# federicobetti99/Conjugate-Gradient

Hardware: AMD Instinct MI355X
Metric: cg_iterations_per_sec (higher is better)
Workload: dtype f64

## Files before the change

conjugate-gradient_amd/cgx.py:

```python
import ctypes as C
import os
import subprocess
import sys

import numpy as np

_PKG = os.path.dirname(os.path.abspath(__file__))
LIB_PATH = os.path.join(_PKG, "libcgx.so")
UNIQUE_ID_BYTES = 128

IPC_HANDLE_BYTES = 64
COMM_SELF, COMM_LOOPBACK, COMM_RCCL, COMM_P2P = 0, 1, 2, 3
MATRIX_DENSE, MATRIX_BANDED = 0, 1
MATRIX_CSR = 2
MAX_DIAGONALS = 64

EXPORTS = [
    "cgx_config_init", "cgx_comm_unique_id", "cgx_create", "cgx_destroy", "cgx_last_error", "cgx_status_string",
    "cgx_get_comm_info", "cgx_get_gemv_plan", "cgx_get_resident_record", "cgx_p2p_export", "cgx_p2p_import", "cgx_p2p_selftest",
    "cgx_partition", "cgx_generate_lap2d_matrix", "cgx_set_matrix_dense", "cgx_read_matrix",
    "cgx_init_source_term", "cgx_set_source_term", "cgx_set_max_iter", "cgx_set_tolerance", "cgx_get_size",
    "cgx_get_matrix_format",
    "cgx_solve", "cgx_solve_begin", "cgx_solve_steps", "cgx_solve_end", "cgx_get_gemv_samples",
    "cgx_get_update_samples",
    "cgx_probe_gemv", "cgx_probe_time_gemv", "cgx_probe_vector_ops", "cgx_probe_get_matrix_rows",
    "cgx_probe_get_source_term", "cgx_probe_set_fault_after", "cgx_probe_set_resident_limit", "cgx_probe_persistent_plan",
    "cgx_probe_parse_matrix_market", "cgx_probe_p2p_mailbox_to_host", "cgx_probe_fill_matrix_hash",
    "cgx_probe_set_p2p_epoch", "cgx_probe_get_p2p_epoch", "cgx_probe_p2p_host_mailboxes", "cgx_probe_resident_test",
    "cgx_solve_multi", "cgx_probe_gemv_multi",
    "cgx_set_preconditioner", "cgx_get_preconditioner",
    "cgx_set_matrix_csr", "cgx_get_matrix_nnz",
]
MAX_RHS = 16
PRECOND_NONE, PRECOND_JACOBI = 0, 1
_PRECOND_NAMES = {None: PRECOND_NONE, "jacobi": PRECOND_JACOBI}


class Config(C.Structure):
    _fields_ = [
        ("struct_version", C.c_int), ("comm_mode", C.c_int), ("device", C.c_int), ("rank", C.c_int),
        ("nranks", C.c_int), ("unique_id", C.c_ubyte * UNIQUE_ID_BYTES), ("gemv_variant", C.c_int),
        ("lda_pad", C.c_int), ("check_every", C.c_int), ("profile_gemv", C.c_int), ("profile_update", C.c_int),
        ("p2p_mailbox_kib", C.c_int), ("p2p_timeout_ms", C.c_int), ("p2p_separate_exchange", C.c_int),
        ("matrix_format", C.c_int), ("profile_first", C.c_int), ("profile_markers", C.c_int),
        ("p2p_no_acquire_fence", C.c_int), ("p2p_tagged", C.c_int),
    ]
# ... 72 lines not shown
        L.cgx_get_matrix_nnz.argtypes = [vp, C.c_int, C.POINTER(C.c_longlong)]
        L.cgx_solve.argtypes = [vp, dp, C.POINTER(Result)]
        L.cgx_solve_begin.argtypes = [vp, dp]
        L.cgx_solve_steps.argtypes = [vp, C.c_int, ip]
        L.cgx_solve_end.argtypes = [vp, dp, C.POINTER(Result)]
        L.cgx_get_gemv_samples.argtypes = [vp, dp, C.c_int, ip]
        L.cgx_get_update_samples.argtypes = [vp, dp, C.c_int, ip]
        L.cgx_probe_gemv.argtypes = [vp, dp, dp, dp]
        L.cgx_probe_time_gemv.argtypes = [vp, C.c_int, dp]
        L.cgx_probe_vector_ops.argtypes = [vp, C.c_int, C.c_double, C.c_double, dp, dp, dp, dp, dp]
        L.cgx_probe_get_matrix_rows.argtypes = [vp, C.c_int, dp, ip, ip]
        L.cgx_probe_get_source_term.argtypes = [vp, C.c_int, dp]
        L.cgx_probe_set_fault_after.argtypes = [vp, C.c_int]
        L.cgx_probe_set_resident_limit.argtypes = [vp, C.c_int]
        L.cgx_probe_persistent_plan.argtypes = [C.c_int, C.c_int, C.c_long, C.c_int, C.POINTER(C.c_long)]
        L.cgx_probe_p2p_mailbox_to_host.argtypes = [vp]
        L.cgx_probe_fill_matrix_hash.argtypes = [vp, C.c_ulonglong, C.c_int, C.c_double]
        L.cgx_probe_p2p_host_mailboxes.argtypes = [vp, C.c_char_p, C.c_int]
        L.cgx_probe_set_p2p_epoch.argtypes = [vp, C.c_int, C.c_ulonglong]
        L.cgx_probe_resident_test.argtypes = [vp, C.c_ulonglong, C.c_int]
        L.cgx_probe_get_p2p_epoch.argtypes = [vp, C.c_int, C.POINTER(C.c_ulonglong)]
        L.cgx_solve_multi.argtypes = [vp, C.c_int, dp, C.c_long, dp, C.c_long, C.POINTER(Result)]
        L.cgx_set_preconditioner.argtypes = [vp, C.c_int]
        L.cgx_get_preconditioner.argtypes = [vp, ip]
        L.cgx_probe_gemv_multi.argtypes = [vp, C.c_int, dp, C.c_long, dp, C.c_long, dp]
        L.cgx_probe_parse_matrix_market.argtypes = [C.c_char_p, C.c_int, ip, ip, ip, ip, ip, ip, dp, C.c_long, C.c_char_p, C.c_int]
        for name in EXPORTS:
            fn = getattr(L, name)
            if fn.restype is C.c_int and name not in ("cgx_config_init",):
                fn.restype = C.c_int
# ... 322 lines not shown
```

conjugate-gradient_amd/csrc/cgx_context.cpp:

```cpp
#include "cgx_internal.h"

#include <sys/mman.h>
#include <sys/stat.h>
#include <fcntl.h>
#include <unistd.h>

#include <algorithm>
#include <cctype>
#include <chrono>
#include <cmath>
#include <cstdio>
#include <cstdlib>
#include <cstring>
#include <string>
#include <vector>

using namespace cgxi;

namespace cgxi {

constexpr int kStreamDefaultMax = 10000;

thread_local std::string g_create_error;

// ... 43 lines not shown
    (void)hipFree(s.A);
    (void)hipFree(s.dia_vals);
    (void)hipFree(s.csr_rp);
    (void)hipFree(s.csr_col);
    (void)hipFree(s.csr_vals);
    (void)hipFree(s.b_full);
    (void)hipFree(s.x);
    (void)hipFree(s.p[0]);
    (void)hipFree(s.p[1]);
    (void)hipFree(s.apg);
    (void)hipFree(s.rbuf);
    (void)hipFree(s.partials);
    (void)hipFree(s.ap_parts);
    (void)hipFree(s.k1_scratch);
    (void)hipFree(s.sym_parts);
    (void)hipFree(s.dinv);
    (void)hipFree(s.zbuf);
    (void)hipFree(s.sc);
    (void)hipFree(s.gathered);
    s = Shard{};
}

void free_problem(cgx_ctx *ctx)
{
    for (auto &s : ctx->shards) free_shard(s);
    ctx->shards.clear();
    (void)hipFree(ctx->d_gathered_ptrs);
    (void)hipFree(ctx->d_scalar_ptrs);
    (void)hipFree(ctx->multi);
    ctx->multi = nullptr;
// ... 129 lines not shown
        ctx->max_iter = n;
        ctx->have_matrix = ctx->have_b = false;
        ctx->in_solve = false;
        for (auto &s : ctx->shards) {
            HIP_TRY(ctx, hipMemsetAsync(s.p[0], 0, (size_t)ctx->lda * sizeof(double), ctx->stream));
            HIP_TRY(ctx, hipMemsetAsync(s.p[1], 0, (size_t)ctx->lda * sizeof(double), ctx->stream));
            HIP_TRY(ctx, hipMemsetAsync(s.sc, 0, sizeof(Scalars), ctx->stream));
            HIP_TRY(ctx, hipMemsetAsync(s.apg, 0, (size_t)ctx->nranks * ctx->seg_S * sizeof(double), ctx->stream));
        }
        {
            int variant = ctx->cfg.gemv_variant;
            if (variant <= 0) {
                const char *e = getenv("CGX_GEMV_VARIANT");
                if (e) variant = atoi(e);
            }
            CGX_TRY(setup_resident(ctx, variant));
        }
        HIP_TRY(ctx, hipStreamSynchronize(ctx->stream));
        return CGX_OK;
    }
    free_problem(ctx);
    ctx->m = ctx->n = n;
    if (n <= (8 << 20) &&
        hipHostMalloc(reinterpret_cast<void **>(&ctx->h_stage), (size_t)(n + 16) * sizeof(double), hipHostMallocDefault) != hipSuccess)
        ctx->h_stage = nullptr;
    ctx->max_iter = n;
    ctx->lda = default_lda(ctx, n);
    ctx->start_rows.assign(ctx->nranks, 0);
    ctx->num_rows.assign(ctx->nranks, 0);
    partition_rows(n, ctx->nranks, ctx->start_rows.data(), ctx->num_rows.data());
    int max_rows = 0;
    for (int q = 0; q < ctx->nranks; ++q) max_rows = std::max(max_rows, ctx->num_rows[q]);
    ctx->seg_Sr = std::max((max_rows + 1) / 2 * 2, 2);

    int variant = ctx->cfg.gemv_variant;
    if (variant <= 0) {
        const char *e = getenv("CGX_GEMV_VARIANT");
        if (e) variant = atoi(e);
    }
    const bool fused_p2p = ctx->cfg.comm_mode == CGX_COMM_P2P && !ctx->cfg.p2p_separate_exchange;
    ctx->chunked = (ctx->nranks > 1 && !ctx->sparse()) || fused_p2p;
    const bool allow_split = ctx->chunked && !ctx->sparse() && ctx->nranks > 1;
    const int k1_variant = (variant == 40000 || variant == 50000) ? 0 : variant;
    auto plan_for = [&](int rows) {
        if (ctx->csr) return cgx::plan_csr(rows, 0, k1_variant);
        return ctx->banded ? cgx::plan_dia(rows, k1_variant) : cgx::plan_gemv(k1_variant, rows, ctx->n, ctx->lda, allow_split);
    };
    int grid_max = 1;
    for (int q = 0; q < ctx->nranks; ++q) {
        const cgx::GemvPlan pl = plan_for(ctx->num_rows[q]);
        grid_max = std::max(grid_max, pl.grid);
        if (pl.split > 1) ctx->chunked = true;
    }
    const int cpr = cgx::chunks_per_rank(ctx->seg_Sr);
// ... 38 lines not shown
    const int seg_tail = (ctx->npart + 1 + 1) / 2 * 2;
    ctx->seg_S = ctx->seg_Sr + seg_tail;
    const int nlocal = (ctx->cfg.comm_mode == CGX_COMM_LOOPBACK) ? ctx->nranks : 1;
    ctx->shards.resize(nlocal);
    for (int i = 0; i < nlocal; ++i) {
        Shard &s = ctx->shards[i];
        s.rank = (ctx->cfg.comm_mode == CGX_COMM_RCCL || ctx->cfg.comm_mode == CGX_COMM_P2P) ? ctx->cfg.rank : i;
        s.row0 = ctx->start_rows[s.rank];
        s.rows = ctx->num_rows[s.rank];
        s.plan = plan_for(s.rows);
        const size_t rows_alloc = (size_t)std::max(s.rows, 1);
        s.npartials = 3 * cgx::update_xr_grid(n) + 8;
        if (!ctx->sparse()) HIP_TRY(ctx, hipMalloc(&s.A, rows_alloc * (size_t)ctx->lda * sizeof(double)));
        HIP_TRY(ctx, hipMalloc(&s.b_full, (size_t)n * sizeof(double)));
        const size_t apg_bytes = (size_t)ctx->nranks * ctx->seg_S * sizeof(double);
        const int rr_parts = cgx::update_xr_grid(n);
        const size_t rbuf_bytes = (size_t)(ctx->lda + rr_parts) * sizeof(double);
        const bool blocks = ctx->cfg.comm_mode == CGX_COMM_SELF && !ctx->sparse();
        HIP_TRY(ctx, hipMalloc(&s.p[0], (size_t)ctx->lda * sizeof(double)));
        if (blocks) {
            static_assert(sizeof(Scalars) <= 16 * sizeof(double), "Scalars must fit the tail of a state block");
            const size_t bytes = (size_t)cgx::state_doubles(ctx->lda) * sizeof(double);
            for (int q = 0; q < 2; ++q) {
                HIP_TRY(ctx, hipMalloc(&s.state[q], bytes));
                HIP_TRY(ctx, hipMemsetAsync(s.state[q], 0, bytes, ctx->stream));
            }
            s.cur = 0;
            bind_state(s, ctx->lda);
        } else {
            HIP_TRY(ctx, hipMalloc(&s.x, rows_alloc * sizeof(double)));
            HIP_TRY(ctx, hipMalloc(&s.p[1], (size_t)ctx->lda * sizeof(double)));
// ... 39 lines not shown
    }
    HIP_TRY(ctx, hipStreamSynchronize(ctx->stream));
    return CGX_OK;
}

cgx_status plan_symmetric(cgx_ctx *ctx)
{
    ctx->dinv_valid = false;
    if (ctx->shards.size() != 1 || ctx->nranks != 1 || ctx->sparse() || ctx->chunked) return CGX_OK;
    Shard &s = ctx->shards[0];
    int variant = ctx->cfg.gemv_variant;
    if (variant <= 0) {
        const char *e = getenv("CGX_GEMV_VARIANT");
        if (e) variant = atoi(e);
    }
    const int k1_variant = (variant == 40000 || variant == 50000) ? 0 : variant;
    const cgx::GemvPlan general = cgx::plan_gemv(k1_variant, s.rows, ctx->n, ctx->lda, false);
    const cgx::GemvPlan sym = cgx::plan_symv(ctx->n, ctx->lda, ctx->cus);
    const bool eligible = variant <= 0 && ctx->n > cgx::kSymvMinN && s.rows == ctx->n && s.A && sym.light <= ctx->npart;
    if (!eligible) {
        s.plan = general;
        return CGX_OK;
    }
    DeviceScratch scratch;
    int *dflag = nullptr;
    HIP_TRY(ctx, scratch.alloc(&dflag, sizeof(int)));
    HIP_TRY(ctx, hipMemsetAsync(dflag, 0, sizeof(int), ctx->stream));
    HIP_TRY(ctx, cgx::launch_symmetric_check(s.A, ctx->lda, ctx->n, dflag, ctx->stream));
    int mismatch = 1;
    HIP_TRY(ctx, hipMemcpyAsync(&mismatch, dflag, sizeof(int), hipMemcpyDeviceToHost, ctx->stream));
    HIP_TRY(ctx, hipStreamSynchronize(ctx->stream));
    if (mismatch) {
        s.plan = general;
        return CGX_OK;
    }
    const size_t bytes = (size_t)sym.split * (size_t)ctx->lda * sizeof(double);
    if (s.sym_parts && s.sym_parts_bytes != bytes) {
        (void)hipFree(s.sym_parts);
        s.sym_parts = nullptr;
        s.sym_parts_bytes = 0;
    }
    if (!s.sym_parts) {
        HIP_TRY(ctx, hipMalloc(&s.sym_parts, bytes));
        s.sym_parts_bytes = bytes;
        HIP_TRY(ctx, hipMemsetAsync(s.sym_parts, 0, bytes, ctx->stream));
        HIP_TRY(ctx, hipStreamSynchronize(ctx->stream));
    }
    s.plan = sym;
    return CGX_OK;
}

}

extern "C" {

void cgx_config_init(cgx_config *cfg)
{
    if (!cfg) return;
    memset(cfg, 0, sizeof *cfg);
    cfg->struct_version = CGX_VERSION;
    cfg->comm_mode = CGX_COMM_SELF;
// ... 433 lines not shown
```

conjugate-gradient_amd/csrc/cgx_internal.h:

```cpp
#pragma once

#include "../../include/cgx.h"

#include <hip/hip_runtime.h>

#include <string>
#include <vector>

#include "cgx_kernels.h"
#include "cgx_rccl.h"

namespace cgxi {

using cgx::Scalars;

struct Shard {
    int rank = 0;
    int row0 = 0;
    int rows = 0;
    double *A = nullptr;
    double *dia_vals = nullptr;
    cgx::DiaView dia{};
    long long *csr_rp = nullptr;
    int *csr_col = nullptr;
    double *csr_vals = nullptr;
    cgx::CsrView csr{};
    double *b_full = nullptr;
    double *state[2] = {nullptr, nullptr};
    int cur = 0;
    double *x = nullptr;
    double *p[2] = {nullptr, nullptr};
    double *apg = nullptr;
    double *rbuf = nullptr;
    double *ap_parts = nullptr;
    double *k1_scratch = nullptr;
    double *partials = nullptr;
    double *sym_parts = nullptr;
    size_t sym_parts_bytes = 0;
    Scalars *sc = nullptr;
    double *gathered = nullptr;
    cgx::GemvPlan plan{};
    cgx::SegView apv{}, rv{};
    double *dinv = nullptr;
    double *zbuf = nullptr;
    cgx::SegView zv{};
    int npartials = 0;
    double *Ap() const { return apg + (size_t)rank * apv.S; }
    double *tail() const { return Ap() + apv.Sr; }
    double *k1_part() const { return k1_scratch ? k1_scratch : tail(); }
};


}
// ... 207 lines not shown
```

conjugate-gradient_amd/csrc/cgx_kernels.h:

```cpp
#pragma once

#include <hip/hip_runtime.h>

namespace cgx {

constexpr int kSlots = 4;
constexpr int kSlotConj = 0;
constexpr int kSlotRr = 1;
constexpr int kSlotX = 2;
constexpr int kMaxRanks = 64;

struct Scalars {
    double rs[2];
    double rr[2];
    double local[kSlots];
    double dbg[4];
    int    done;
    int    k_final;
    unsigned pad[2];
};

struct SegView {
    double *base;
    int S, Sr;
// ... 6 lines not shown
};

void seg_finalize(SegView *sv);

struct GemvPlan {
    int variant;
    int R;
    int U;
    int waves;
    int nt;
    int grid;
    int rows_per_wg;
    int ncols;
    int split;
    int light;
};

GemvPlan plan_gemv(int variant, int rows, int n, long lda, bool allow_split = false);

hipError_t launch_gemv_plain(const GemvPlan &plan, const double *A, long lda, int rows, const double *v_full,
                             const double *v_local, double *Ap, double *partials, Scalars *sc, hipStream_t s);

hipError_t launch_gemv_fused(const GemvPlan &plan, const double *A, long lda, int rows, int row0,
                             const double *p_old, double *p_new, SegView seg, double *Ap, double *partials,
                             Scalars *sc, int k, double tol, hipStream_t s, hipEvent_t e_start = nullptr,
                             hipEvent_t e_stop = nullptr, long ap_stride = 0, bool jacobi = false);
constexpr int kSymvTile = 256;
constexpr int kSymvMinN = 16384;
GemvPlan plan_symv(int n, long lda, int cus);
inline int plan_partials(const GemvPlan &pl) { return pl.variant == 6 ? pl.light : pl.grid / (pl.split > 1 ? pl.split : 1); }
hipError_t launch_symv_plain(const GemvPlan &pl, const double *A, long lda, int n, const double *v, double *parts, double *Ap,
                             double *partials, hipStream_t s);
hipError_t launch_symv_fused(const GemvPlan &pl, const double *A, long lda, int n, const double *p_old, double *p_new, SegView seg,
                             double *parts, double *Ap, double *partials, Scalars *sc, int k, double tol, hipStream_t s,
                             hipEvent_t e_start = nullptr, hipEvent_t e_stop = nullptr, bool jacobi = false);
hipError_t launch_symmetric_check(const double *A, long lda, int n, int *mismatch, hipStream_t s);

constexpr int kChunkRows = 512;
inline int chunks_per_rank(int Sr) { return (Sr + kChunkRows - 1) / kChunkRows; }
hipError_t launch_prefold_ap(const double *parts, int split, long stride, int rows, int Sr, const double *p_loc, double *dst,
                             double *tail, const Scalars *sc, hipStream_t s);

hipError_t launch_update_xr(int n, int rows, int row0, const double *p_new, SegView apv, int tail_off, int tail_count,
                            double *x, SegView rv, Scalars *sc, int parity, double *partials, hipStream_t s,
                            hipEvent_t e_start = nullptr, hipEvent_t e_stop = nullptr,
                            const double *dinv = nullptr, SegView zv = SegView{});
int update_xr_grid(int count);
constexpr int kMaxVectorGrid = 1024;

hipError_t launch_close_iteration(Scalars *sc, SegView seg, int k, double tol, hipStream_t s, bool jacobi = false);
// ... 203 lines not shown
```

conjugate-gradient_amd/csrc/cgx_probe.cpp:

```cpp
#include "cgx_internal.h"

#include <fcntl.h>
#include <sys/mman.h>
#include <sys/stat.h>
#include <unistd.h>

#include <algorithm>
#include <cctype>
#include <chrono>
#include <cmath>
#include <cstdio>
#include <cstdlib>
#include <cstring>
#include <string>
#include <vector>

using namespace cgxi;

extern "C" {

cgx_status cgx_probe_gemv(cgx_ctx *ctx, const double *p, double *y, double *pAp)
{
    if (!ctx || !p || !y) return fail(ctx, CGX_ERR_BAD_ARG, "cgx_probe_gemv: bad argument");
    if (!ctx->have_matrix) return fail(ctx, CGX_ERR_BAD_ARG, "no matrix");
// ... 238 lines not shown
    ctx->p2p_ready = true;
    return CGX_OK;
}

cgx_status cgx_probe_persistent_plan(int n, int cus, long lds_per_cu, int streaming, long out[CGX_PERSISTENT_PLAN_INTS])
{
    if (!out || n < 1 || cus < 1 || lds_per_cu < 0) return CGX_ERR_BAD_ARG;
    cgx::ResidentPlan pl{};
    const bool fits = streaming ? cgx::plan_stream(n, cus, (size_t)lds_per_cu, &pl) : cgx::plan_resident(n, cus, (size_t)lds_per_cu, &pl);
    const long r[CGX_PERSISTENT_PLAN_INTS] = {fits ? 1 : 0, pl.R, pl.S, pl.grid, pl.xslots, (long)pl.lds_bytes, pl.RL, pl.RG, pl.RB, pl.l2_rows,
                                              pl.hybrid, pl.stream ? 512 : 256};
    for (int i = 0; i < CGX_PERSISTENT_PLAN_INTS; ++i) out[i] = fits || i == 0 ? r[i] : 0;
    return CGX_OK;
}

cgx_status cgx_probe_set_resident_limit(cgx_ctx *ctx, int workgroups)
{
    if (!ctx) return CGX_ERR_BAD_ARG;
    ctx->resident_limit = workgroups;
    return CGX_OK;
}

cgx_status cgx_probe_get_source_term(cgx_ctx *ctx, int local_shard, double *b_out)
{
    if (!ctx || !b_out || local_shard < 0 || local_shard >= (int)ctx->shards.size())
        return fail(ctx, CGX_ERR_BAD_ARG, "cgx_probe_get_source_term: bad argument");
    if (!ctx->have_b) return fail(ctx, CGX_ERR_BAD_ARG, "no source term");
    HIP_TRY(ctx, hipSetDevice(ctx->device));
    HIP_TRY(ctx, hipMemcpy(b_out, ctx->shards[local_shard].b_full, (size_t)ctx->n * sizeof(double), hipMemcpyDeviceToHost));
    return CGX_OK;
// ... 55 lines not shown
```

conjugate-gradient_amd/csrc/cgx_solve.cpp:

```cpp
#include "cgx_internal.h"

#include <sys/file.h>

#include <cerrno>
#include <climits>
#include <thread>

#include <algorithm>
#include <cctype>
#include <chrono>
#include <cmath>
#include <cstdio>
#include <cstdlib>
#include <cstring>
#include <string>
#include <vector>

using namespace cgxi;

namespace cgxi {


cgx_status p2p_allgather(cgx_ctx *ctx, int chan, const double *src, int count, double *dst, long dst_stride,
                         int copy_self, int tail_off, int tail_n, int sum_off)
// ... 60 lines not shown
cgx_status prepare_jacobi(cgx_ctx *ctx)
{
    if (ctx->banded) return fail(ctx, CGX_ERR_UNSUPPORTED, "Jacobi preconditioner: banded storage is not supported");
    if (ctx->res_forced)
        return fail(ctx, CGX_ERR_UNSUPPORTED, "Jacobi preconditioner: the persistent kernels (gemv_variant 40000 / 50000) have no Jacobi form");
    hipStream_t st = ctx->stream;
    for (auto &s : ctx->shards) {
        if (!s.dinv) {
            const size_t zbytes = (size_t)(s.rv.S + (s.rv.S - s.rv.Sr)) * sizeof(double);
            HIP_TRY(ctx, hipMalloc(&s.dinv, (size_t)ctx->lda * sizeof(double)));
            HIP_TRY(ctx, hipMalloc(&s.zbuf, zbytes));
            HIP_TRY(ctx, hipMemsetAsync(s.zbuf, 0, zbytes, st));
        }
        s.zv = s.rv;
        s.zv.base = s.zbuf;
    }
    if (ctx->dinv_valid) return CGX_OK;
    for (auto &s : ctx->shards) {
        if (ctx->csr)
            HIP_TRY(ctx, cgx::launch_csr_diag_slice(s.csr, s.rows, s.row0, s.Ap(), st));
        else
            HIP_TRY(ctx, cgx::launch_diag_slice(s.A, ctx->lda, s.rows, s.row0, s.Ap(), st));
    }
    CGX_TRY(gather_segments(ctx, false));
    if (!ctx->d_jbad) HIP_TRY(ctx, hipMalloc(reinterpret_cast<void **>(&ctx->d_jbad), sizeof(int)));
    HIP_TRY(ctx, hipMemsetAsync(ctx->d_jbad, 0x7f, sizeof(int), st));
    for (auto &s : ctx->shards) HIP_TRY(ctx, cgx::launch_jacobi_dinv(s.apv, ctx->n, ctx->lda, s.dinv, ctx->d_jbad, st));
    int bad = INT_MAX;
    HIP_TRY(ctx, hipMemcpyAsync(&bad, ctx->d_jbad, sizeof(int), hipMemcpyDeviceToHost, st));
    HIP_TRY(ctx, hipStreamSynchronize(st));
// ... 39 lines not shown
    *e1 = ctx->upd_pool[ctx->upd_used++];
    return CGX_OK;
}

}

namespace cgxi {

cgx_status run_gemv_plain(cgx_ctx *ctx, Shard &s, const double *v_full)
{
    if (ctx->csr)
        HIP_TRY(ctx, cgx::launch_spmv_csr_plain(s.plan, s.csr, s.rows, s.row0, ctx->lda, v_full, s.Ap(), s.k1_part(), ctx->stream));
    else if (ctx->banded)
        HIP_TRY(ctx, cgx::launch_spmv_dia_plain(s.plan, s.dia, s.rows, s.row0, ctx->n, ctx->lda, v_full, s.Ap(), s.k1_part(), s.sc,
                                                ctx->stream));
    else if (s.plan.variant == 6)
        HIP_TRY(ctx, cgx::launch_symv_plain(s.plan, s.A, ctx->lda, ctx->n, v_full, s.sym_parts, s.Ap(), s.k1_part(), ctx->stream));
    else
        HIP_TRY(ctx, cgx::launch_gemv_plain(s.plan, s.A, ctx->lda, s.rows, v_full, v_full + s.row0, s.Ap(), s.k1_part(),
                                            s.sc, ctx->stream));
    return CGX_OK;
}

cgx_status run_gemv_fused(cgx_ctx *ctx, Shard &s, int k)
{
    const int every = ctx->cfg.profile_gemv;
    const long long seq = ctx->gemv_seq++;
    bool timed = false;
    if (every > 0 && ctx->ev_used + 2 <= 4096) {
        if (seq == 0) {
// ... 9 lines not shown
        CGX_TRY(take_event(ctx, &e0));
        CGX_TRY(take_event(ctx, &e1));
        if (ctx->cfg.profile_markers) {
            HIP_TRY(ctx, hipEventRecord(e0, ctx->stream));
            e0 = e1 = nullptr;
        }
    }
    hipEvent_t m1 = (timed && ctx->cfg.profile_markers) ? ctx->ev_pool[ctx->ev_used - 1] : nullptr;
    const bool pc = ctx->precond == CGX_PRECOND_JACOBI;
    if (ctx->csr)
        HIP_TRY(ctx, cgx::launch_spmv_csr_fused(s.plan, s.csr, s.rows, s.row0, ctx->lda, s.p[k & 1], s.p[(k + 1) & 1], pc ? s.zv : s.rv,
                                                s.Ap(), s.k1_part(), s.sc, k, ctx->tol, ctx->stream, e0, e1, pc));
    else if (ctx->banded)
        HIP_TRY(ctx, cgx::launch_spmv_dia_fused(s.plan, s.dia, s.rows, s.row0, ctx->n, ctx->lda, s.p[k & 1], s.p[(k + 1) & 1],
                                                s.rv, s.Ap(), s.k1_part(), s.sc, k, ctx->tol, ctx->stream, e0, e1));
    else if (s.plan.variant == 6)
        HIP_TRY(ctx, cgx::launch_symv_fused(s.plan, s.A, ctx->lda, ctx->n, s.p[k & 1], s.p[(k + 1) & 1], pc ? s.zv : s.rv, s.sym_parts,
                                            s.Ap(), s.k1_part(), s.sc, k, ctx->tol, ctx->stream, e0, e1, pc));
    else
        HIP_TRY(ctx, cgx::launch_gemv_fused(s.plan, s.A, ctx->lda, s.rows, s.row0, s.p[k & 1], s.p[(k + 1) & 1], pc ? s.zv : s.rv,
                                            s.plan.split > 1 ? s.ap_parts : s.Ap(),
                                            (ctx->chunked && s.plan.light) ? nullptr : s.k1_part(),
                                            s.sc, k, ctx->tol, ctx->stream, e0, e1, ctx->seg_Sr, pc));
    if (m1) HIP_TRY(ctx, hipEventRecord(m1, ctx->stream));
    return CGX_OK;
}

void reset_gemv_stats(cgx_ctx *ctx)
{
    ctx->ev_used = 0;
// ... 49 lines not shown
        HIP_TRY(ctx, cgx::launch_update_xr_p2p(ctx->n, s.rows, s.row0, s.p[(k + 1) & 1], s.apv, ctx->npart, ctx->mv, 1, epoch,
                                               s.x, s.rv, s.sc, k & 1, ctx->p2p_timeout_ticks, ctx->d_p2p_err, st,
                                               s.plan.split > 1 ? s.ap_parts : s.Ap(), s.plan.split, ctx->seg_Sr, u0, u1,
                                               pc ? s.dinv : nullptr, s.zv));
        return CGX_OK;
    }
    if (ctx->chunked)
        for (auto &s : ctx->shards)
            HIP_TRY(ctx, cgx::launch_prefold_ap(s.plan.split > 1 ? s.ap_parts : s.Ap(), s.plan.split, ctx->seg_Sr, s.rows, ctx->seg_Sr,
                                                s.p[(k + 1) & 1] + s.row0, s.Ap(), s.tail(), s.sc, st));
    CGX_TRY(gather_segments(ctx, true));
    const bool folded = ctx->cfg.comm_mode == CGX_COMM_P2P;
    for (auto &s : ctx->shards) {
        hipEvent_t u0 = nullptr, u1 = nullptr;
        if (&s == &ctx->shards[0]) CGX_TRY(take_update_events(ctx, &u0, &u1));
        const int count = folded ? 1 : (s.plan.variant == 6 ? cgx::plan_partials(s.plan) : ctx->npart);
        HIP_TRY(ctx, cgx::launch_update_xr(ctx->n, s.rows, s.row0, s.p[(k + 1) & 1], s.apv, folded ? ctx->npart : 0,
                                           count, s.x, s.rv, s.sc, k & 1, s.partials, st, u0, u1,
                                           pc ? s.dinv : nullptr, s.zv));
    }
    return CGX_OK;
}

cgx_status check_p2p_error(cgx_ctx *ctx)
{
    if (ctx->cfg.comm_mode != CGX_COMM_P2P || !ctx->d_p2p_err) return CGX_OK;
    int e = 0;
    HIP_TRY(ctx, hipMemcpy(&e, ctx->d_p2p_err, sizeof(int), hipMemcpyDeviceToHost));
    if (e) return fail(ctx, CGX_ERR_P2P, "direct peer exchange: a wait for a peer's flag expired (peer dead or IPC not coherent)");
    return CGX_OK;
// ... 443 lines not shown
```

include/cgx.h:

```cpp
#ifndef CGX_H
#define CGX_H

#ifdef __cplusplus
extern "C" {
#endif

#define CGX_VERSION 1
#define CGX_UNIQUE_ID_BYTES 128
#define CGX_IPC_HANDLE_BYTES 64

typedef enum cgx_status {
    CGX_OK = 0,
    CGX_ERR_BAD_ARG = 1,
    CGX_ERR_IO = 2,
    CGX_ERR_HIP = 3,
    CGX_ERR_RCCL = 4,
    CGX_ERR_OOM = 5,
    CGX_ERR_NO_DEVICE = 6,
    CGX_ERR_UNSUPPORTED = 7,
    CGX_ERR_P2P = 8
} cgx_status;

typedef enum cgx_comm_mode {
    CGX_COMM_SELF = 0,
// ... 103 lines not shown
cgx_status  cgx_solve_multi(cgx_ctx *ctx, int nrhs, const double *B, long ldb, double *X, long ldx, cgx_result *res);
cgx_status  cgx_probe_gemv_multi(cgx_ctx *ctx, int nrhs, const double *P, long ldp, double *Y, long ldy, double *pAp);

cgx_status  cgx_probe_gemv(cgx_ctx *ctx, const double *p, double *y, double *pAp);
cgx_status  cgx_probe_time_gemv(cgx_ctx *ctx, int reps, double *ms_per_launch);
cgx_status  cgx_probe_vector_ops(cgx_ctx *ctx, int n, double alpha, double beta, double *x, double *r,
                                 double *p, const double *Ap, double *rr);
cgx_status  cgx_probe_set_fault_after(cgx_ctx *ctx, int calls);
cgx_status  cgx_probe_parse_matrix_market(const char *path, int threads, int *m, int *n, int *nz, int *symmetric, int *I, int *J,
                                          double *a, long cap, char *err, int err_cap);
cgx_status  cgx_probe_p2p_mailbox_to_host(cgx_ctx *ctx);
cgx_status  cgx_probe_p2p_host_mailboxes(cgx_ctx *ctx, const char *prefix, int stage);
cgx_status  cgx_probe_set_resident_limit(cgx_ctx *ctx, int workgroups);
#define CGX_PERSISTENT_PLAN_INTS 12
cgx_status  cgx_probe_persistent_plan(int n, int cus, long lds_per_cu, int streaming, long out[CGX_PERSISTENT_PLAN_INTS]);
cgx_status  cgx_probe_set_p2p_epoch(cgx_ctx *ctx, int chan, unsigned long long value);
cgx_status  cgx_probe_get_p2p_epoch(cgx_ctx *ctx, int chan, unsigned long long *value);
cgx_status  cgx_probe_resident_test(cgx_ctx *ctx, unsigned long long epoch, int mute_workgroup);
cgx_status  cgx_probe_get_source_term(cgx_ctx *ctx, int local_shard, double *b_out);
cgx_status  cgx_probe_fill_matrix_hash(cgx_ctx *ctx, unsigned long long seed, int symmetric, double diag);
cgx_status  cgx_probe_get_matrix_rows(cgx_ctx *ctx, int local_shard, double *A_out, int *row0, int *rows);

#ifdef __cplusplus
}
#endif
#endif
```

Before: 1369.

## Add evenly balanced symmetric SYMV tile schedule with fold-into-update kernel

Adds a new symmetric matrix-vector path that splits the upper-triangle tile work into equal-length step runs across a fixed grid of four workgroups per CU, so no workgroup gets a heavier share. Tiles that are cut between workgroups write their column sums to an extras buffer, looked up through a host-built table. The x/r update kernel then folds the per-strip partial results directly, removing a separate reduction pass. This is the default for single-rank dense problems above the size threshold, with variant 60000 keeping the old chain path. The price is extra buffers and more complex indexing, plus correctness risk around tiles that are split between workgroups.

After: 1369. About the same (-0.0%).

```diff
diff --git a/conjugate-gradient_amd/cgx.py b/conjugate-gradient_amd/cgx.py
--- a/conjugate-gradient_amd/cgx.py
+++ b/conjugate-gradient_amd/cgx.py
@@ -30,6 +30,7 @@
     "cgx_solve_multi", "cgx_probe_gemv_multi",
     "cgx_set_preconditioner", "cgx_get_preconditioner",
     "cgx_set_matrix_csr", "cgx_get_matrix_nnz",
+    "cgx_probe_symv_even_plan",
 ]
 MAX_RHS = 16
 PRECOND_NONE, PRECOND_JACOBI = 0, 1
@@ -132,6 +133,7 @@
         L.cgx_probe_set_fault_after.argtypes = [vp, C.c_int]
         L.cgx_probe_set_resident_limit.argtypes = [vp, C.c_int]
         L.cgx_probe_persistent_plan.argtypes = [C.c_int, C.c_int, C.c_long, C.c_int, C.POINTER(C.c_long)]
+        L.cgx_probe_symv_even_plan.argtypes = [C.c_int, C.c_int, C.c_int, C.c_int, C.POINTER(C.c_longlong), C.POINTER(C.c_longlong), ip]
         L.cgx_probe_p2p_mailbox_to_host.argtypes = [vp]
         L.cgx_probe_fill_matrix_hash.argtypes = [vp, C.c_ulonglong, C.c_int, C.c_double]
         L.cgx_probe_p2p_host_mailboxes.argtypes = [vp, C.c_char_p, C.c_int]
diff --git a/conjugate-gradient_amd/csrc/cgx_context.cpp b/conjugate-gradient_amd/csrc/cgx_context.cpp
--- a/conjugate-gradient_amd/csrc/cgx_context.cpp
+++ b/conjugate-gradient_amd/csrc/cgx_context.cpp
@@ -81,6 +81,8 @@
     (void)hipFree(s.ap_parts);
     (void)hipFree(s.k1_scratch);
     (void)hipFree(s.sym_parts);
+    (void)hipFree(s.sym_extras);
+    (void)hipFree(s.sym_xtab);
     (void)hipFree(s.dinv);
     (void)hipFree(s.zbuf);
     (void)hipFree(s.sc);
@@ -240,6 +242,7 @@
                 const char *e = getenv("CGX_GEMV_VARIANT");
                 if (e) variant = atoi(e);
             }
+            if (variant == cgx::kSymvChainVariant) variant = 0;
             CGX_TRY(setup_resident(ctx, variant));
         }
         HIP_TRY(ctx, hipStreamSynchronize(ctx->stream));
@@ -264,6 +267,7 @@
         const char *e = getenv("CGX_GEMV_VARIANT");
         if (e) variant = atoi(e);
     }
+    if (variant == cgx::kSymvChainVariant) variant = 0;
     const bool fused_p2p = ctx->cfg.comm_mode == CGX_COMM_P2P && !ctx->cfg.p2p_separate_exchange;
     ctx->chunked = (ctx->nranks > 1 && !ctx->sparse()) || fused_p2p;
     const bool allow_split = ctx->chunked && !ctx->sparse() && ctx->nranks > 1;
@@ -332,7 +336,12 @@
         if (!ctx->sparse()) HIP_TRY(ctx, hipMalloc(&s.A, rows_alloc * (size_t)ctx->lda * sizeof(double)));
         HIP_TRY(ctx, hipMalloc(&s.b_full, (size_t)n * sizeof(double)));
         const size_t apg_bytes = (size_t)ctx->nranks * ctx->seg_S * sizeof(double);
-        const int rr_parts = cgx::update_xr_grid(n);
+        int rr_parts = cgx::update_xr_grid(n);
+        {
+            const int even_parts = (ctx->seg_Sr + cgx::kSymvEvenRows - 1) / cgx::kSymvEvenRows;
+            if (ctx->nranks == 1 && !ctx->sparse() && n > cgx::kSymvMinN && even_parts <= (int)cgx::kStateTail)
+                rr_parts = std::max(rr_parts, even_parts);
+        }
         const size_t rbuf_bytes = (size_t)(ctx->lda + rr_parts) * sizeof(double);
         const bool blocks = ctx->cfg.comm_mode == CGX_COMM_SELF && !ctx->sparse();
         HIP_TRY(ctx, hipMalloc(&s.p[0], (size_t)ctx->lda * sizeof(double)));
@@ -402,9 +411,11 @@
         const char *e = getenv("CGX_GEMV_VARIANT");
         if (e) variant = atoi(e);
     }
+    const bool chain = variant == cgx::kSymvChainVariant;
+    if (chain) variant = 0;
     const int k1_variant = (variant == 40000 || variant == 50000) ? 0 : variant;
     const cgx::GemvPlan general = cgx::plan_gemv(k1_variant, s.rows, ctx->n, ctx->lda, false);
-    const cgx::GemvPlan sym = cgx::plan_symv(ctx->n, ctx->lda, ctx->cus);
+    cgx::GemvPlan sym = cgx::plan_symv(ctx->n, ctx->lda, ctx->cus);
     const bool eligible = variant <= 0 && ctx->n > cgx::kSymvMinN && s.rows == ctx->n && s.A && sym.light <= ctx->npart;
     if (!eligible) {
         s.plan = general;
@@ -433,6 +444,27 @@
         s.sym_parts_bytes = bytes;
         HIP_TRY(ctx, hipMemsetAsync(s.sym_parts, 0, bytes, ctx->stream));
         HIP_TRY(ctx, hipStreamSynchronize(ctx->stream));
+    }
+    cgx::GemvPlan even{};
+    if (!chain && s.state[0] && cgx::plan_symv_even(ctx->n, ctx->lda, ctx->cus, ctx->npart, s.rv.S - s.rv.Sr, &even)) {
+        if (!s.sym_xtab || s.sym_even_grid != even.grid) {
+            (void)hipFree(s.sym_extras);
+            (void)hipFree(s.sym_xtab);
+            s.sym_extras = nullptr;
+            s.sym_xtab = nullptr;
+            std::vector<int> host((size_t)even.split + 1 + (size_t)even.grid);
+            cgx::SymvEvenTable tab;
+            tab.offsets = host.data();
+            if (!cgx::plan_symv_even_table(ctx->n, even.grid, &tab)) return fail(ctx, CGX_ERR_UNSUPPORTED, "symmetric K1: no even plan");
+            const size_t xbytes = (size_t)even.grid * cgx::kSymvTile * sizeof(double);
+            HIP_TRY(ctx, hipMalloc(&s.sym_extras, xbytes));
+            HIP_TRY(ctx, hipMalloc(&s.sym_xtab, host.size() * sizeof(int)));
+            HIP_TRY(ctx, hipMemsetAsync(s.sym_extras, 0, xbytes, ctx->stream));
+            HIP_TRY(ctx, hipMemcpyAsync(s.sym_xtab, host.data(), host.size() * sizeof(int), hipMemcpyHostToDevice, ctx->stream));
+            HIP_TRY(ctx, hipStreamSynchronize(ctx->stream));
+            s.sym_even_grid = even.grid;
+        }
+        sym = even;
     }
     s.plan = sym;
     return CGX_OK;
diff --git a/conjugate-gradient_amd/csrc/cgx_internal.h b/conjugate-gradient_amd/csrc/cgx_internal.h
--- a/conjugate-gradient_amd/csrc/cgx_internal.h
+++ b/conjugate-gradient_amd/csrc/cgx_internal.h
@@ -37,6 +37,9 @@
     double *partials = nullptr;
     double *sym_parts = nullptr;
     size_t sym_parts_bytes = 0;
+    double *sym_extras = nullptr;
+    int *sym_xtab = nullptr;
+    int sym_even_grid = 0;
     Scalars *sc = nullptr;
     double *gathered = nullptr;
     cgx::GemvPlan plan{};
diff --git a/conjugate-gradient_amd/csrc/cgx_kernels.h b/conjugate-gradient_amd/csrc/cgx_kernels.h
--- a/conjugate-gradient_amd/csrc/cgx_kernels.h
+++ b/conjugate-gradient_amd/csrc/cgx_kernels.h
@@ -44,6 +44,7 @@
     int ncols;
     int split;
     int light;
+    int even;
 };
 
 GemvPlan plan_gemv(int variant, int rows, int n, long lda, bool allow_split = false);
@@ -58,12 +59,37 @@
 constexpr int kSymvTile = 256;
 constexpr int kSymvMinN = 16384;
 GemvPlan plan_symv(int n, long lda, int cus);
-inline int plan_partials(const GemvPlan &pl) { return pl.variant == 6 ? pl.light : pl.grid / (pl.split > 1 ? pl.split : 1); }
+inline int plan_partials(const GemvPlan &pl)
+{
+    if (pl.variant == 6) return pl.even ? pl.grid : pl.light;
+    return pl.grid / (pl.split > 1 ? pl.split : 1);
+}
 hipError_t launch_symv_plain(const GemvPlan &pl, const double *A, long lda, int n, const double *v, double *parts, double *Ap,
                              double *partials, hipStream_t s);
 hipError_t launch_symv_fused(const GemvPlan &pl, const double *A, long lda, int n, const double *p_old, double *p_new, SegView seg,
                              double *parts, double *Ap, double *partials, Scalars *sc, int k, double tol, hipStream_t s,
                              hipEvent_t e_start = nullptr, hipEvent_t e_stop = nullptr, bool jacobi = false);
+constexpr int kSymvSteps = 8;
+constexpr int kSymvChainVariant = 60000;
+constexpr int kSymvEvenRows = 128;
+struct SymvEvenTable {
+    int nb = 0, grid = 0;
+    long steps = 0;
+    int max_run = 0, min_run = 0;
+    int entries = 0;
+    int *offsets = nullptr;
+};
+bool plan_symv_even_table(int n, int G, SymvEvenTable *tab);
+bool plan_symv_even(int n, long lda, int cus, int tail_capacity, int rr_capacity, GemvPlan *out);
+hipError_t launch_symv_even_plain(const GemvPlan &pl, const double *A, long lda, int n, const double *v, double *parts,
+                                  double *extras, const int *xtab, double *Ap, double *partials, hipStream_t s);
+hipError_t launch_symv_even_fused(const GemvPlan &pl, const double *A, long lda, int n, const double *p_old, double *p_new,
+                                  SegView seg, double *parts, double *extras, double *partials, Scalars *sc, int k, double tol,
+                                  hipStream_t s, hipEvent_t e_start = nullptr, hipEvent_t e_stop = nullptr, bool jacobi = false);
+hipError_t launch_symv_even_update(const GemvPlan &pl, int n, long lda, const double *parts, const double *extras, const int *xtab,
+                                   const double *p_new, const double *partials, double *x, SegView rv, Scalars *sc, int parity,
+                                   hipStream_t s, hipEvent_t e_start = nullptr, hipEvent_t e_stop = nullptr,
+                                   const double *dinv = nullptr, SegView zv = SegView{});
 hipError_t launch_symmetric_check(const double *A, long lda, int n, int *mismatch, hipStream_t s);
 
 constexpr int kChunkRows = 512;
diff --git a/conjugate-gradient_amd/csrc/cgx_probe.cpp b/conjugate-gradient_amd/csrc/cgx_probe.cpp
--- a/conjugate-gradient_amd/csrc/cgx_probe.cpp
+++ b/conjugate-gradient_amd/csrc/cgx_probe.cpp
@@ -276,6 +276,26 @@
     return CGX_OK;
 }
 
+cgx_status cgx_probe_symv_even_plan(int n, int grid, int tail_capacity, int rr_capacity, long long out[CGX_SYMV_EVEN_PLAN_INTS],
+                                    long long *starts, int *table)
+{
+    if (!out || n < 1 || grid < 1 || grid % 4 != 0) return CGX_ERR_BAD_ARG;
+    cgx::SymvEvenTable tab;
+    tab.offsets = table;
+    const bool cut = cgx::plan_symv_even_table(n, grid, &tab);
+    cgx::GemvPlan pl{};
+    const long lda = ((long)n + 15) / 16 * 16 + 16;
+    const bool even = cut && cgx::plan_symv_even(n, lda, grid / 4, tail_capacity, rr_capacity, &pl);
+    const long long tiles = (long long)tab.nb * (tab.nb + 1) / 2;
+    const long long r[CGX_SYMV_EVEN_PLAN_INTS] = {even ? 1 : 0, tab.nb, tiles, tab.steps, tab.min_run, tab.max_run, tab.entries,
+                                                  even ? pl.light : 0};
+    for (int i = 0; i < CGX_SYMV_EVEN_PLAN_INTS; ++i) out[i] = r[i];
+    if (even && (pl.grid != grid || pl.U != tab.max_run)) return CGX_ERR_UNSUPPORTED;
+    if (starts)
+        for (int g = 0; g <= grid; ++g) starts[g] = (long long)(tab.steps * g / grid);
+    return CGX_OK;
+}
+
 cgx_status cgx_probe_set_resident_limit(cgx_ctx *ctx, int workgroups)
 {
     if (!ctx) return CGX_ERR_BAD_ARG;
diff --git a/conjugate-gradient_amd/csrc/cgx_solve.cpp b/conjugate-gradient_amd/csrc/cgx_solve.cpp
--- a/conjugate-gradient_amd/csrc/cgx_solve.cpp
+++ b/conjugate-gradient_amd/csrc/cgx_solve.cpp
@@ -98,6 +98,7 @@
         }
         s.zv = s.rv;
         s.zv.base = s.zbuf;
+        HIP_TRY(ctx, hipMemsetAsync(s.zbuf + s.rv.Sr, 0, (size_t)(2 * (s.rv.S - s.rv.Sr)) * sizeof(double), st));
     }
     if (ctx->dinv_valid) return CGX_OK;
     for (auto &s : ctx->shards) {
@@ -167,6 +168,9 @@
     else if (ctx->banded)
         HIP_TRY(ctx, cgx::launch_spmv_dia_plain(s.plan, s.dia, s.rows, s.row0, ctx->n, ctx->lda, v_full, s.Ap(), s.k1_part(), s.sc,
                                                 ctx->stream));
+    else if (s.plan.variant == 6 && s.plan.even)
+        HIP_TRY(ctx, cgx::launch_symv_even_plain(s.plan, s.A, ctx->lda, ctx->n, v_full, s.sym_parts, s.sym_extras, s.sym_xtab, s.Ap(),
+                                                 s.k1_part(), ctx->stream));
     else if (s.plan.variant == 6)
         HIP_TRY(ctx, cgx::launch_symv_plain(s.plan, s.A, ctx->lda, ctx->n, v_full, s.sym_parts, s.Ap(), s.k1_part(), ctx->stream));
     else
@@ -206,6 +210,9 @@
     else if (ctx->banded)
         HIP_TRY(ctx, cgx::launch_spmv_dia_fused(s.plan, s.dia, s.rows, s.row0, ctx->n, ctx->lda, s.p[k & 1], s.p[(k + 1) & 1],
                                                 s.rv, s.Ap(), s.k1_part(), s.sc, k, ctx->tol, ctx->stream, e0, e1));
+    else if (s.plan.variant == 6 && s.plan.even)
+        HIP_TRY(ctx, cgx::launch_symv_even_fused(s.plan, s.A, ctx->lda, ctx->n, s.p[k & 1], s.p[(k + 1) & 1], pc ? s.zv : s.rv,
+                                                 s.sym_parts, s.sym_extras, s.k1_part(), s.sc, k, ctx->tol, ctx->stream, e0, e1, pc));
     else if (s.plan.variant == 6)
         HIP_TRY(ctx, cgx::launch_symv_fused(s.plan, s.A, ctx->lda, ctx->n, s.p[k & 1], s.p[(k + 1) & 1], pc ? s.zv : s.rv, s.sym_parts,
                                             s.Ap(), s.k1_part(), s.sc, k, ctx->tol, ctx->stream, e0, e1, pc));
@@ -285,6 +292,11 @@
     for (auto &s : ctx->shards) {
         hipEvent_t u0 = nullptr, u1 = nullptr;
         if (&s == &ctx->shards[0]) CGX_TRY(take_update_events(ctx, &u0, &u1));
+        if (s.plan.variant == 6 && s.plan.even) {
+            HIP_TRY(ctx, cgx::launch_symv_even_update(s.plan, ctx->n, ctx->lda, s.sym_parts, s.sym_extras, s.sym_xtab, s.p[(k + 1) & 1],
+                                                      s.k1_part(), s.x, s.rv, s.sc, k & 1, st, u0, u1, pc ? s.dinv : nullptr, s.zv));
+            continue;
+        }
         const int count = folded ? 1 : (s.plan.variant == 6 ? cgx::plan_partials(s.plan) : ctx->npart);
         HIP_TRY(ctx, cgx::launch_update_xr(ctx->n, s.rows, s.row0, s.p[(k + 1) & 1], s.apv, folded ? ctx->npart : 0,
                                            count, s.x, s.rv, s.sc, k & 1, s.partials, st, u0, u1,
diff --git a/conjugate-gradient_amd/csrc/cgx_symv_even.hip b/conjugate-gradient_amd/csrc/cgx_symv_even.hip
--- /dev/null
+++ b/conjugate-gradient_amd/csrc/cgx_symv_even.hip
@@ -0,0 +1,413 @@
+#include "cgx_kernels.h"
+#include "cgx_device.h"
+
+#include <hip/hip_ext.h>
+
+#include <vector>
+
+namespace cgx {
+
+namespace {
+
+constexpr int kB = kSymvTile;
+constexpr int kEvenWaves = 8;
+
+__device__ __forceinline__ long even_strip_start(long I, long nb) { return I * nb - I * (I - 1) / 2; }
+__device__ __forceinline__ void even_tile(long t, long nb, long *I, long *J)
+{
+    const double b = 2.0 * (double)nb + 1.0;
+    long i = (long)((b - sqrt(b * b - 8.0 * (double)t)) * 0.5);
+    i = i < 0 ? 0 : (i > nb - 1 ? nb - 1 : i);
+    while (i + 1 < nb && even_strip_start(i + 1, nb) <= t) ++i;
+    while (i > 0 && even_strip_start(i, nb) > t) --i;
+    *I = i;
+    *J = i + (t - even_strip_start(i, nb));
+}
+
+}
+
+template <bool FUSED, bool PRE>
+__global__ __launch_bounds__(256, 4) void k_symv_even_tiles(const double *__restrict__ A, long lda, int n, int ncols, int nb, long steps,
+                                                            const double *__restrict__ v, double *__restrict__ p_new, SegView sv,
+                                                            double *__restrict__ parts, double *__restrict__ extras,
+                                                            double *__restrict__ tail, Scalars *sc, int k, double tol)
+{
+    constexpr int B = kB;
+    constexpr int H = B / 128;
+    constexpr int R = 16 / H;
+    constexpr int RW = B / 4;
+    static_assert(H == 2 && R == 8 && RW == 64 && RW / R == kSymvSteps, "a step is one batch of the four waves");
+    __shared__ double rowbuf[2][B];
+    __shared__ double colbuf[2][4][B];
+    __shared__ double red[4];
+
+    const int lane = threadIdx.x & 63, w = threadIdx.x >> 6;
+    const long G = gridDim.x;
+    const long s0 = steps * (long)blockIdx.x / G, s1 = steps * ((long)blockIdx.x + 1) / G;
+    double beta = 0.0;
+    if constexpr (FUSED) {
+        const HeadLoadsOf<PRE> hl = head_issue_t<PRE>(sc, sv, k);
+        const IterHead h = head_finish_t<PRE>(hl, sc, sv, k, tol);
+        if (hl.done || h.stop) return;
+        beta = h.beta;
+    }
+    if (s0 >= s1) return;
+    const long t0 = s0 / kSymvSteps, tl = (s1 - 1) / kSymvSteps;
+    long I, J;
+    even_tile(t0, nb, &I, &J);
+    const double *rfull = sv.base;
+
+    auto vec2 = [&](int c) {
+        const bool ok = c < ncols;
+        const int cc = ok ? c : 0;
+        d2 p = *reinterpret_cast<const d2 *>(v + cc);
+        if constexpr (FUSED) {
+            const d2 r = *reinterpret_cast<const d2 *>(rfull + cc);
+            p.x = fma(beta, p.x, r.x);
+            p.y = fma(beta, p.y, r.y);
+        }
+        p.x = ok ? p.x : 0.0;
+        p.y = ok ? p.y : 0.0;
+        return p;
+    };
+    auto vec1 = [&](int i) {
+        const bool ok = i < n;
+        const int ii = ok ? i : 0;
+        double p = v[ii];
+        if constexpr (FUSED) p = fma(beta, p, rfull[ii]);
+        return ok ? p : 0.0;
+    };
+
+    const int e = threadIdx.x;
+    const int eb = lane >> 3;
+    double pap = 0.0;
+    int buf = 0;
+    for (long t = t0; t <= tl; ++t) {
+        const int b_lo = t == t0 ? (int)(s0 - t0 * kSymvSteps) : 0;
+        const int b_hi = t == tl ? (int)(s1 - tl * kSymvSteps) : kSymvSteps;
+        const int r0 = (int)(I * B), c0 = (int)(J * B);
+        const bool diag = I == J;
+        int col[H];
+        d2 pj[H];
+#pragma unroll
+        for (int h = 0; h < H; ++h) {
+            col[h] = c0 + h * 128 + 2 * lane;
+            pj[h] = vec2(col[h]);
+            if constexpr (FUSED)
+                if (diag && b_lo == 0 && w == 0 && col[h] < ncols) *reinterpret_cast<d2 *>(p_new + col[h]) = pj[h];
+            if (col[h] >= ncols) col[h] = ncols - 2;
+        }
+        const double pi_l = vec1(r0 + w * RW + lane);
+        d2 cacc[H];
+#pragma unroll
+        for (int h = 0; h < H; ++h) cacc[h] = d2{0.0, 0.0};
+
+        for (int b = b_lo; b < b_hi; ++b) {
+            const int rb = r0 + w * RW + b * R;
+            d2 a[R][H];
+#pragma unroll
+            for (int q = 0; q < R; ++q) {
+                long row = rb + q;
+                if (row > n - 1) row = n - 1;
+                const char *ar = reinterpret_cast<const char *>(A + row * lda);
+#pragma unroll
+                for (int h = 0; h < H; ++h) a[q][h] = load_a<true>(reinterpret_cast<const double *>(ar + (unsigned)col[h] * 8u));
+            }
+            __builtin_amdgcn_sched_barrier(0);
+            double racc[R];
+#pragma unroll
+            for (int q = 0; q < R; ++q) {
+                racc[q] = fma(a[q][0].y, pj[0].y, a[q][0].x * pj[0].x);
+#pragma unroll
+                for (int h = 1; h < H; ++h) racc[q] = fma(a[q][h].y, pj[h].y, fma(a[q][h].x, pj[h].x, racc[q]));
+                const int src = b * R + q;
+                const double pr = __hiloint2double(__builtin_amdgcn_readlane(__double2hiint(pi_l), src),
+                                                   __builtin_amdgcn_readlane(__double2loint(pi_l), src));
+#pragma unroll
+                for (int h = 0; h < H; ++h) {
+                    cacc[h].x = fma(a[q][h].x, pr, cacc[h].x);
+                    cacc[h].y = fma(a[q][h].y, pr, cacc[h].y);
+                }
+            }
+            const int myrow = wave_sum_rows<R>(racc, lane);
+            if ((lane & (64 / R - 1)) == 0) rowbuf[buf][w * RW + b * R + myrow] = racc[0];
+        }
+        if (!diag)
+#pragma unroll
+            for (int h = 0; h < H; ++h) *reinterpret_cast<d2 *>(&colbuf[buf][w][h * 128 + 2 * lane]) = cacc[h];
+        __syncthreads();
+        if (eb >= b_lo && eb < b_hi && r0 + e < n) {
+            const double rp = rowbuf[buf][e];
+            parts[J * lda + r0 + e] = rp;
+            pap = fma(diag ? pi_l : 2.0 * pi_l, rp, pap);
+        }
+        if (!diag && c0 + e < n) {
+            const double cs = ((colbuf[buf][0][e] + colbuf[buf][1][e]) + colbuf[buf][2][e]) + colbuf[buf][3][e];
+            if (b_lo == 0) parts[I * lda + c0 + e] = cs;
+            else extras[(long)blockIdx.x * B + e] = cs;
+        }
+        buf ^= 1;
+        if (++J == nb) { ++I; J = I; }
+    }
+    pap = block_sum<4>(pap, red);
+    if (threadIdx.x == 0) tail[blockIdx.x] = pap;
+}
+
+namespace {
+
+struct EvenLds {
+    d2 red[kEvenWaves][64];
+    d2 xred[kEvenWaves][64];
+    double cs[kEvenWaves];
+};
+
+__device__ __forceinline__ d2 even_row_pair(const double *__restrict__ parts, long lda, int nb, const double *__restrict__ extras,
+                                            const int *__restrict__ xtab, int rc, int J, double cs_wave, EvenLds &L)
+{
+    const int lane = threadIdx.x & 63, w = threadIdx.x >> 6;
+    const int x0 = xtab[J], x1 = xtab[J + 1];
+    const int s0 = nb * w / kEvenWaves, s1 = nb * (w + 1) / kEvenWaves;
+    d2 acc{0.0, 0.0};
+    for (int s = s0; s < s1; s += 8) {
+        d2 x[8];
+#pragma unroll
+        for (int u = 0; u < 8; ++u) {
+            const int su = s + u < s1 ? s + u : s1 - 1;
+            x[u] = *reinterpret_cast<const d2 *>(parts + (long)su * lda + rc);
+        }
+#pragma unroll
+        for (int u = 0; u < 8; ++u) {
+            acc.x = s + u < s1 ? acc.x + x[u].x : acc.x;
+            acc.y = s + u < s1 ? acc.y + x[u].y : acc.y;
+        }
+    }
+    const int ne = x1 - x0;
+    const int q0 = x0 + ne * w / kEvenWaves, q1 = x0 + ne * (w + 1) / kEvenWaves;
+    const int *list = xtab + nb + 1;
+    d2 xacc{0.0, 0.0};
+    for (int q = q0; q < q1; q += 4) {
+        d2 x[4];
+#pragma unroll
+        for (int u = 0; u < 4; ++u) {
+            const int g = list[q + u < q1 ? q + u : q1 - 1];
+            x[u] = *reinterpret_cast<const d2 *>(extras + (long)g * kB + (rc & (kB - 1)));
+        }
+#pragma unroll
+        for (int u = 0; u < 4; ++u) {
+            xacc.x = q + u < q1 ? xacc.x + x[u].x : xacc.x;
+            xacc.y = q + u < q1 ? xacc.y + x[u].y : xacc.y;
+        }
+    }
+    L.red[w][lane] = acc;
+    L.xred[w][lane] = xacc;
+    if (lane == 0) L.cs[w] = cs_wave;
+    __syncthreads();
+    d2 a{0.0, 0.0};
+    if (w == 0) {
+        a = L.red[0][lane];
+#pragma unroll
+        for (int i = 1; i < kEvenWaves; ++i) {
+            a.x += L.red[i][lane].x;
+            a.y += L.red[i][lane].y;
+        }
+#pragma unroll
+        for (int i = 0; i < kEvenWaves; ++i) {
+            a.x += L.xred[i][lane].x;
+            a.y += L.xred[i][lane].y;
+        }
+    }
+    return a;
+}
+
+}
+
+__global__ __launch_bounds__(kEvenWaves * 64) void k_symv_even_fold(const double *__restrict__ parts, long lda, int nb, int Sr,
+                                                                    const double *__restrict__ extras, const int *__restrict__ xtab,
+                                                                    double *__restrict__ Ap)
+{
+    __shared__ EvenLds L;
+    const int lane = threadIdx.x & 63;
+    const int row = (int)blockIdx.x * kSymvEvenRows + 2 * lane;
+    const int rc = row < Sr ? row : 0;
+    const int J = ((int)blockIdx.x * kSymvEvenRows) / kB;
+    const d2 a = even_row_pair(parts, lda, nb, extras, xtab, rc, J, 0.0, L);
+    if (threadIdx.x < 64 && row < Sr) *reinterpret_cast<d2 *>(Ap + row) = a;
+}
+
+template <bool PRE>
+__global__ __launch_bounds__(kEvenWaves * 64) void k_symv_even_update(const double *__restrict__ parts, long lda, int nb, int n, int Sr,
+                                                                      const double *__restrict__ extras, const int *__restrict__ xtab,
+                                                                      const double *__restrict__ p_new, const double *__restrict__ tail,
+                                                                      int G, double *__restrict__ x, SegView rv, Scalars *sc, int parity,
+                                                                      const double *__restrict__ dinv, SegView zv)
+{
+    __shared__ EvenLds L;
+    double *r = rv.base;
+    const int lane = threadIdx.x & 63, w = threadIdx.x >> 6;
+    const int done = sc->done;
+    const double rsold = sc->rs[parity];
+    const int row = (int)blockIdx.x * kSymvEvenRows + 2 * lane;
+    const int rc = row < Sr ? row : 0;
+    const int J = ((int)blockIdx.x * kSymvEvenRows) / kB;
+    d2 pv{0.0, 0.0}, xv{0.0, 0.0}, rvv{0.0, 0.0}, dv{0.0, 0.0};
+    if (w == 0) {
+        pv = *reinterpret_cast<const d2 *>(p_new + rc);
+        xv = *reinterpret_cast<const d2 *>(x + rc);
+        rvv = *reinterpret_cast<const d2 *>(r + rc);
+        if constexpr (PRE) dv = *reinterpret_cast<const d2 *>(dinv + rc);
+    }
+    double cs = 0.0;
+    for (int f = threadIdx.x; f < G; f += 4 * kEvenWaves * 64) {
+        double a[4];
+#pragma unroll
+        for (int u = 0; u < 4; ++u) {
+            const int g = f + u * kEvenWaves * 64;
+            const double val = tail[g < G ? g : G - 1];
+            a[u] = g < G ? val : 0.0;
+        }
+        cs += (a[0] + a[1]) + (a[2] + a[3]);
+    }
+    cs = wave_sum(cs);
+    const d2 a = even_row_pair(parts, lda, nb, extras, xtab, rc, J, cs, L);
+    if (w != 0) return;
+    double conj = L.cs[0];
+#pragma unroll
+    for (int i = 1; i < kEvenWaves; ++i) conj += L.cs[i];
+    const double alpha = safeguarded_alpha(rsold, conj);
+    const bool in0 = row < n, in1 = row + 1 < n;
+    const bool st = !done && in0;
+    d2 xn, rn;
+    xn.x = fma(alpha, pv.x, xv.x);
+    xn.y = in1 ? fma(alpha, pv.y, xv.y) : xv.y;
+    double rr = 0.0, rz = 0.0;
+    if constexpr (PRE) {
+        const PcRow o0 = pc_update_row(alpha, a.x, rvv.x, dv.x), o1 = pc_update_row(alpha, a.y, rvv.y, dv.y);
+        rn = d2{o0.r, in1 ? o1.r : rvv.y};
+        const d2 zn{o0.z, in1 ? o1.z : 0.0};
+        rr = (in0 ? o0.rr : 0.0) + (in1 ? o1.rr : 0.0);
+        rz = (in0 ? o0.rz : 0.0) + (in1 ? o1.rz : 0.0);
+        if (st) *reinterpret_cast<d2 *>(zv.base + row) = zn;
+    } else {
+        const double r0n = fma(-alpha, a.x, rvv.x), r1n = fma(-alpha, a.y, rvv.y);
+        rn = d2{r0n, in1 ? r1n : rvv.y};
+        rr = (in0 ? r0n * r0n : 0.0) + (in1 ? r1n * r1n : 0.0);
+    }
+    if (st) {
+        *reinterpret_cast<d2 *>(x + row) = xn;
+        *reinterpret_cast<d2 *>(r + row) = rn;
+    }
+    rr = wave_sum(rr);
+    if constexpr (PRE) {
+        rz = wave_sum(rz);
+        if (!done && lane == 0) pc_store_partials(zv, blockIdx.x, rz, rr);
+    } else {
+        if (!done && lane == 0) r[rv.Sr + blockIdx.x] = rr;
+    }
+}
+
+bool plan_symv_even_table(int n, int G, SymvEvenTable *tab)
+{
+    if (n < 1 || G < 1 || !tab) return false;
+    const int nb = (n + kB - 1) / kB;
+    const long tiles = (long)nb * (nb + 1) / 2, steps = tiles * kSymvSteps;
+    tab->nb = nb;
+    tab->grid = G;
+    tab->steps = steps;
+    tab->min_run = (int)(steps / G);
+    tab->max_run = (int)((steps + G - 1) / G);
+    tab->entries = 0;
+    if (tab->min_run < kSymvSteps) return false;
+    std::vector<int> block(G, -1);
+    std::vector<int> count(nb + 1, 0);
+    long I = 0, strip = 0;
+    for (int g = 0; g < G; ++g) {
+        const long s0 = steps * g / G;
+        if (s0 % kSymvSteps == 0) continue;
+        const long t = s0 / kSymvSteps;
+        while (t >= strip + (nb - I)) { strip += nb - I; ++I; }
+        const long J = I + (t - strip);
+        if (J == I) continue;
+        block[g] = (int)J;
+        ++count[J];
+        ++tab->entries;
+    }
+    if (!tab->offsets) return true;
+    int *off = tab->offsets, *list = tab->offsets + nb + 1;
+    off[0] = 0;
+    for (int j = 0; j < nb; ++j) off[j + 1] = off[j] + count[j];
+    std::vector<int> fill(off, off + nb);
+    for (int g = 0; g < G; ++g)
+        if (block[g] >= 0) list[fill[block[g]]++] = g;
+    for (int q = tab->entries; q < G; ++q) list[q] = 0;
+    return true;
+}
+
+bool plan_symv_even(int n, long lda, int cus, int tail_capacity, int rr_capacity, GemvPlan *out)
+{
+    GemvPlan pl = plan_symv(n, lda, cus);
+    const int G = 4 * (cus > 0 ? cus : 256);
+    SymvEvenTable tab;
+    if (!plan_symv_even_table(n, G, &tab)) return false;
+    const int Sr = (n + 1) / 2 * 2;
+    pl.light = (Sr + kSymvEvenRows - 1) / kSymvEvenRows;
+    if (G > tail_capacity || pl.light > rr_capacity) return false;
+    pl.grid = G;
+    pl.U = tab.max_run;
+    pl.even = 1;
+    *out = pl;
+    return true;
+}
+
+namespace {
+
+template <bool FUSED, bool PRE>
+hipError_t launch_even_tiles(const GemvPlan &pl, const double *A, long lda, int n, const double *v, double *p_new, SegView sv,
+                             double *parts, double *extras, double *tail, Scalars *sc, int k, double tol, hipStream_t s, hipEvent_t e0,
+                             hipEvent_t e1)
+{
+    if (pl.variant != 6 || !pl.even || pl.R != kB || n < 2 || !parts || !extras || !tail) return hipErrorInvalidValue;
+    const long steps = (long)pl.split * (pl.split + 1) / 2 * kSymvSteps;
+    if (steps / pl.grid < kSymvSteps) return hipErrorInvalidValue;
+    hipExtLaunchKernelGGL((k_symv_even_tiles<FUSED, PRE>), dim3(pl.grid), dim3(256), 0, s, e0, e1, 0, A, lda, n, pl.ncols, pl.split,
+                          steps, v, p_new, sv, parts, extras, tail, sc, k, tol);
+    return hipGetLastError();
+}
+
+}
+
+hipError_t launch_symv_even_plain(const GemvPlan &pl, const double *A, long lda, int n, const double *v, double *parts,
+                                  double *extras, const int *xtab, double *Ap, double *partials, hipStream_t s)
+{
+    hipError_t e = launch_even_tiles<false, false>(pl, A, lda, n, v, nullptr, SegView{}, parts, extras, partials, nullptr, 0, 0.0, s,
+                                                   nullptr, nullptr);
+    if (e != hipSuccess) return e;
+    const int Sr = (n + 1) / 2 * 2;
+    hipLaunchKernelGGL(k_symv_even_fold, dim3(pl.light), dim3(kEvenWaves * 64), 0, s, parts, lda, pl.split, Sr, extras, xtab, Ap);
+    return hipGetLastError();
+}
+
+hipError_t launch_symv_even_fused(const GemvPlan &pl, const double *A, long lda, int n, const double *p_old, double *p_new,
+                                  SegView seg, double *parts, double *extras, double *partials, Scalars *sc, int k, double tol,
+                                  hipStream_t s, hipEvent_t e_start, hipEvent_t e_stop, bool jacobi)
+{
+    if (jacobi)
+        return launch_even_tiles<true, true>(pl, A, lda, n, p_old, p_new, seg, parts, extras, partials, sc, k, tol, s, e_start, e_stop);
+    return launch_even_tiles<true, false>(pl, A, lda, n, p_old, p_new, seg, parts, extras, partials, sc, k, tol, s, e_start, e_stop);
+}
+
+hipError_t launch_symv_even_update(const GemvPlan &pl, int n, long lda, const double *parts, const double *extras, const int *xtab,
+                                   const double *p_new, const double *partials, double *x, SegView rv, Scalars *sc, int parity,
+                                   hipStream_t s, hipEvent_t e_start, hipEvent_t e_stop, const double *dinv, SegView zv)
+{
+    if (pl.variant != 6 || !pl.even || rv.S - rv.Sr < pl.light) return hipErrorInvalidValue;
+    const int Sr = (n + 1) / 2 * 2;
+    if (dinv)
+        hipExtLaunchKernelGGL((k_symv_even_update<true>), dim3(pl.light), dim3(kEvenWaves * 64), 0, s, e_start, e_stop, 0, parts, lda,
+                              pl.split, n, Sr, extras, xtab, p_new, partials, pl.grid, x, rv, sc, parity, dinv, zv);
+    else
+        hipExtLaunchKernelGGL((k_symv_even_update<false>), dim3(pl.light), dim3(kEvenWaves * 64), 0, s, e_start, e_stop, 0, parts, lda,
+                              pl.split, n, Sr, extras, xtab, p_new, partials, pl.grid, x, rv, sc, parity, dinv, zv);
+    return hipGetLastError();
+}
+
+}
diff --git a/include/cgx.h b/include/cgx.h
--- a/include/cgx.h
+++ b/include/cgx.h
@@ -141,6 +141,9 @@
 cgx_status  cgx_probe_set_resident_limit(cgx_ctx *ctx, int workgroups);
 #define CGX_PERSISTENT_PLAN_INTS 12
 cgx_status  cgx_probe_persistent_plan(int n, int cus, long lds_per_cu, int streaming, long out[CGX_PERSISTENT_PLAN_INTS]);
+#define CGX_SYMV_EVEN_PLAN_INTS 8
+cgx_status  cgx_probe_symv_even_plan(int n, int grid, int tail_capacity, int rr_capacity, long long out[CGX_SYMV_EVEN_PLAN_INTS],
+                                     long long *starts, int *table);
 cgx_status  cgx_probe_set_p2p_epoch(cgx_ctx *ctx, int chan, unsigned long long value);
 cgx_status  cgx_probe_get_p2p_epoch(cgx_ctx *ctx, int chan, unsigned long long *value);
 cgx_status  cgx_probe_resident_test(cgx_ctx *ctx, unsigned long long epoch, int mute_workgroup);
```
